# Vipermaseg/libagmv

Measured on AMD Instinct MI355X. Metric: frames/s encode+decode (AGMV hot path: quantise+classify+assemble, parse+reconstruct), synthetic, higher is better.
Workload: dtype u8; 1 GPU; c3: 1024-frame 1920x1080 agmv_synth_v1, HIGH_QUALITY palette, OPT_III (512 colours); frames_per_gpu=1024, width=1920, height=1080, palette=512 colours, reference histogram build (GPU histogram + host pick), parallelism=1024 frames per rank, 1 rank(s), no data-path collective

## Files before the change

libagmv_amd/csrc/agmv_decode_hip.hip:

```cpp
#include <hip/hip_runtime.h>

#include <stdint.h>
#include <stdlib.h>
#include <string.h>
#include <type_traits>

#include "agmv_hip_impl.h"

#ifndef DEC_T_OVERRIDE
#define DEC_T_OVERRIDE 256
#endif
constexpr int DEC_T = DEC_T_OVERRIDE;
#ifndef DEC_BPB
#define DEC_BPB 24
#endif
constexpr int DEC_STAGE = DEC_T * DEC_BPB;
constexpr int DEC_SR = DEC_STAGE / 4 / DEC_T;
constexpr int DEC_MAX_SLICES = 32;

struct dec_ws {
	uint32_t* d_dirty;
	size_t dirty_cap;
	bool dep_split;
	uint32_t* d_parse_ws;
	size_t parse_ws_cap;
	uint32_t* d_fp_ws;
	size_t fp_ws_cap;
	uint32_t* d_fp_fstate;
	uint32_t fp_frames;
	uint32_t* d_nent_own;
	size_t nent_cap;
	hipStream_t aux_stream;
	hipEvent_t ev_fork;
	hipEvent_t ev_slice[DEC_MAX_SLICES];
};

static dec_ws* dec_area(agmv_hip_ctx* c) { return (dec_ws*)c->ws[AREA_DEC]; }

static void dec_free(void* p)
{
	dec_ws* d = (dec_ws*)p;
	(void)hipFree(d->d_dirty); (void)hipFree(d->d_parse_ws); (void)hipFree(d->d_fp_ws); (void)hipFree(d->d_nent_own);
	if (d->ev_fork) (void)hipEventDestroy(d->ev_fork);
	for (int i = 0; i < DEC_MAX_SLICES; i++) if (d->ev_slice[i]) (void)hipEventDestroy(d->ev_slice[i]);
	if (d->aux_stream) (void)hipStreamDestroy(d->aux_stream);
	free(d);
}

static int need_dec_ctx(agmv_hip_ctx* c, bool palette)
{
	if (agmv_hip_enter(c, palette)) return -1;
	return palette && !agmv_hip_area(c, AREA_DEC, sizeof(dec_ws), dec_free) ? -1 : 0;
}

template <class F>
static void dec_flags(F&& f) { f(); }
template <class F, class... Rest>
static void dec_flags(F&& f, bool flag, Rest... rest) { dec_flags([&](auto... r_) { if (flag) f(std::true_type(), r_...); else f(std::false_type(), r_...); }, rest...); }
#define DEC_LAUNCH(k, grid, block, s, A, ...) do { \
	dec_flags([&](auto... b_) { hipLaunchKernelGGL((k<decltype(b_)::value...>), grid, block, 0, s, A); }, __VA_ARGS__); \
	CK(hipGetLastError()); } while (0)

__device__ __forceinline__ bool is_flag(uint32_t b) { return b == FILL_FLAG || b == NORMAL_FLAG || b == COPY_FLAG; }

struct ByteSrc {
	const uint8_t* p;
	uint32_t cap;
	__device__ __forceinline__ uint32_t operator()(uint32_t pos) const { return pos < cap ? p[pos] : 0u; }
};

struct StagedSrc {
	const __attribute__((address_space(3))) uint8_t* lds;
	uint32_t lo, len;
	const uint8_t* p;
	uint32_t cap;
	__device__ __forceinline__ uint32_t operator()(uint32_t pos) const
	{
		const uint32_t d = pos - lo;
		if (d < len) return lds[d];
		return pos < cap ? p[pos] : 0u;
	}
};

__global__ __launch_bounds__(64) void k_parse_serial(const uint8_t* __restrict__ bits, unsigned long long stride,
                                                     const uint32_t* __restrict__ bpos_a, uint32_t n_frames,
                                                     uint32_t nblk, int mode512, uint32_t* __restrict__ offsets,
                                                     uint32_t* __restrict__ nentered)
{
	uint32_t f = blockIdx.x * 64u + threadIdx.x;
	if (f >= n_frames) return;
	ByteSrc src{bits + (size_t)f * stride, (uint32_t)stride};
	const uint32_t bpos = bpos_a[f];
	uint32_t* off = offsets + (size_t)f * nblk;
	uint32_t bitpos = 0, k = 0;
	bool escape = false;
	while (k < nblk && !escape) {
		if (bitpos > bpos) break;
		off[k++] = bitpos;
		uint32_t byte = src(bitpos++);
		bool invalid = false;
		while (!is_flag(byte)) {
			byte = src(bitpos++);
			if (bitpos > bpos) { escape = true; break; }
		}
		if (!is_flag(byte)) invalid = true;
		if (byte == FILL_FLAG) {
			uint32_t idx = src(bitpos++);
			if (mode512 && (idx & 0x7fu) == 127u) bitpos++;
			if (bitpos > bpos) escape = true;
		} else if (byte == COPY_FLAG) {
		} else {
			for (int j = 0; j < 4; j++)
				for (int i = 0; i < 4; i++) {
					uint32_t idx = src(bitpos++);
					if (mode512 && (idx & 0x7fu) == 127u) bitpos++;
					if (bitpos > bpos || invalid) { escape = true; invalid = false; break; }
				}
		}
	}
	nentered[f] = k;
}

constexpr int PC = 512;
constexpr int PNSEG = PC / 64;
#ifndef PEL_OVERRIDE
#define PEL_OVERRIDE 3
#endif
constexpr int PCL = 3;
constexpr int PEL = PEL_OVERRIDE;
constexpr int PHALO = 64;
constexpr uint32_t J_EXIT = 0x8000u;
constexpr uint32_t J_END = 0xFFFFu;
constexpr uint32_t X_END = 63u;

constexpr int FC = 64;
constexpr int FH = 4;
constexpr int FOWN = 64 - FH - 1;
constexpr int FRB = FOWN * FC;

struct ParseArgs {
	const uint8_t* bits;
	unsigned long long stride;
	const uint32_t* bpos;
	uint32_t cpf;
	uint16_t* summ;
	uint32_t* centry;
	uint32_t* offsets;
	uint32_t* nentered;
	uint32_t n_frames, nblk;
	const uint32_t* fstate;
	const uint32_t* nbad;
	unsigned long long* vm;
	uint32_t maxR;
};
constexpr uint32_t FS_OK = 0, FS_TODO = 1, FS_BAD = 2;

__device__ __forceinline__ uint32_t parse_nch(const ParseArgs& A, uint32_t f, uint32_t bpos)
{
	return (!A.fstate || A.fstate[f] == FS_BAD) ? (bpos + PC) / PC : 0u;
}

__device__ __forceinline__ void wave_lds_sync()
{
	__builtin_amdgcn_fence(__ATOMIC_ACQ_REL, "wavefront");
	__builtin_amdgcn_wave_barrier();
}

template <int NLV>
struct ParseLds {
	uint8_t b[PC + PHALO];
	unsigned long long esc[PNSEG + 2];
	uint16_t jl[NLV][PC];
};

constexpr int PCD = ((PC + PHALO) / 4 + 63) / 64;

__device__ __forceinline__ void load_chunk(uint32_t (&raw)[PCD], const uint8_t* fbits, uint32_t cap, uint32_t cs, int lane)
{
#pragma unroll
	for (int q = 0; q < PCD; q++) {
		const uint32_t pos = cs + 4u * (uint32_t)(q * 64 + lane);
		raw[q] = (q * 64 + lane < (PC + PHALO) / 4 && pos < cap) ? *(const uint32_t*)(fbits + pos) : 0u;
	}
}

template <bool M512, int NLV>
__device__ __forceinline__ uint32_t parse_chunk_nodes(ParseLds<NLV>& S, uint16_t* rank_at, uint16_t* npos, uint16_t* eo, uint16_t* n0,
                                                      const uint32_t (&raw)[PCD], uint32_t bpos, uint32_t cs, int lane)
{
#pragma unroll
	for (int q = 0; q < PCD; q++) {
		const int i = q * 64 + lane;
		if (i < (PC + PHALO) / 4) ((uint32_t*)S.b)[i] = raw[q];
	}
	wave_lds_sync();
// ... 1026 lines not shown
			for (int k = 0; k < 16; k++) icol[k] = cur[k];
			istale = stale;
		}
		anystale |= stale != 0;
		if (!needfix) depstale |= stale != 0;
		if (valid) store_block(A.out + (size_t)f * npx, poff, A.w, cur);
	}
	if (valid && (anystale || needfix)) {
		if (group != 0 || needfix) {
			atomicOr(A.dirty + (blk >> 5), 1u << (blk & 31u));
			A.dirty[(A.nblk + 31) >> 5] = 1u;
		}
		if (group == 0 && depstale) A.dirty[((A.nblk + 31) >> 5) + 1] = 1u;
	}
	if (!LOOP) break;
	item += gridDim.x;
	if (item >= A.n_items) break;
	__syncthreads();
	}
}

template <bool M512, bool BM>
__global__ __launch_bounds__(64) void k_fixup(DecArgs A)
{
	__shared__ uint32_t s_pal[512];
	const int lane = threadIdx.x;
	const uint32_t npx = A.w * A.h;
	const uint32_t nwords = (A.nblk + 31) >> 5;
	if (A.dirty[nwords] == 0) return;
	const uint32_t base = blockIdx.x * 64u;
	const uint32_t w0 = A.dirty[base >> 5], w1 = (base >> 5) + 1 < nwords ? A.dirty[(base >> 5) + 1] : 0u;
	if ((w0 | w1) == 0) return;
	uint32_t blk = base + (uint32_t)lane;
	bool active = blk < A.nblk && (((lane < 32 ? w0 : w1) >> (lane & 31)) & 1u);
	const uint32_t last = A.nblk - 1;
	const bool have_last = last >= base && last < base + 64 && ((((last - base) < 32 ? w0 : w1) >> ((last - base) & 31)) & 1u);
	int nb_lane = -1;
	if (have_last && A.nblk >= 2) {
		if (last > base) { nb_lane = (int)(last - base) - 1; if (lane == nb_lane) active = true; }
		else { nb_lane = 1; if (lane == 1) { blk = last - 1; active = true; } }
	}
	for (int i = lane; i < 512; i += 64) s_pal[i] = A.pal[i];
	__syncthreads();
	if (!active) blk = 0;
	const uint32_t by = blk / A.bw, bx = blk - by * A.bw;
	const uint32_t poff = by * 4 * A.w + bx * 4;
	const bool is_last = active && blk == last;
	uint32_t cur[16], icol[16];
	if (A.prev) load_block(A.prev, poff, A.w, cur);
	else {
#pragma unroll
		for (int k = 0; k < 16; k++) cur[k] = 0;
	}
	if (A.prev_iframe) load_block(A.prev_iframe, poff, A.w, icol);
	else {
#pragma unroll
		for (int k = 0; k < 16; k++) icol[k] = 0;
	}
	uint32_t stale = 0xFFFFu, istale = 0xFFFFu;
	bool dep = false;
	for (uint32_t f = 0; f < A.n_frames; f++) {
		bool fill_written = false;
		const uint32_t own3 = cur[3], own3s = (stale >> 3) & 1u;
		if (active && blk < A.nentered[f]) {
			ByteSrc src{A.bits + (size_t)f * A.stride, (uint32_t)A.stride};
			const uint32_t o = BM ? bm_offset_of(A.vm, A.kb, A.maxR, A.bpos[f], f, blk) : A.offsets[(size_t)f * A.nblk + blk];
			decode_block<M512>(src, o, A.bpos[f], s_pal, cur, icol, istale, stale, fill_written);
		}
		const int nbl = nb_lane < 0 ? 0 : nb_lane;
		const uint32_t left = (uint32_t)__builtin_amdgcn_readlane((int)cur[7], nbl);
		const uint32_t lefts = ((uint32_t)__builtin_amdgcn_readlane((int)stale, nbl) >> 7) & 1u;
		if (is_last && fill_written) {
			const uint32_t c = A.bw == 1 ? own3 : left;
#pragma unroll
			for (int k = 0; k < 16; k++) cur[k] = c;
			stale = (A.bw == 1 ? own3s : lefts) ? 0xFFFFu : 0u;
		}
		if (((A.first_fc + f) & 3u) == 0) {
#pragma unroll
			for (int k = 0; k < 16; k++) icol[k] = cur[k];
			istale = stale;
		}
		if (active) store_block(A.out + (size_t)f * npx, poff, A.w, cur);
		if (active && stale) dep = true;
	}
	if (dep) A.dirty[nwords + 1] = 1u;
}

static int check_slab(const uint8_t* d_bits, size_t stride)
{
	if ((stride & 3u) || stride < 4 || ((uintptr_t)d_bits & 3u)) return agmv_hip_err("agmv_hip: bitstream slab and stride must be 4-byte aligned");
	return 0;
}

struct DecRows {
	const uint8_t* bits;
	size_t stride;
	const uint32_t* bpos;
	uint32_t *offsets, *nentered;
	uint32_t n_frames, nblk;
};
static DecRows rows_range(DecRows r, uint32_t f0, uint32_t f1)
{
	r.bits += (size_t)f0 * r.stride; r.bpos += f0; r.nentered += f0; r.n_frames = f1 - f0;
	if (r.offsets) r.offsets += (size_t)f0 * r.nblk;
	return r;
}
struct DecPix {
	uint32_t w, h, first_fc;
	uint32_t* out;
	const uint32_t *prev, *prev_iframe;
};

static uint32_t dirty_words(uint32_t nblk) { return (nblk + 31) / 32 + 2; }

enum ParseMode { PARSE_FAST, PARSE_ROBUST, PARSE_SERIAL };
static ParseMode parse_mode()
{
	const char* m = getenv("AGMV_HIP_PARSE");
	return !m ? PARSE_FAST : strcmp(m, "robust") == 0 ? PARSE_ROBUST : strcmp(m, "serial") == 0 ? PARSE_SERIAL : PARSE_FAST;
}

static uint32_t parse_grid_x(agmv_hip_ctx* c, uint32_t n_frames, size_t cap)
{
	uint32_t gx = (uint32_t)(((size_t)c->n_cu * 512 + n_frames - 1) / n_frames);
	if (gx < 32) gx = 32;
	if (gx > 256) gx = 256;
	if (gx > cap) gx = (uint32_t)cap;
	return gx < 1 ? 1 : gx;
}

static int parse_launch_robust(agmv_hip_ctx* c, const DecRows& r, size_t ws_frames, hipStream_t s,
                               const uint32_t* fstate, const uint32_t* nbad, unsigned long long* vm, uint32_t maxR)
{
	const size_t cpf = (r.stride + PC) / PC, maxchunks = cpf * ws_frames;
	if (maxchunks >> 32) return agmv_hip_err("agmv_hip: parser batch too large (%zu chunk rows)", maxchunks);
	dec_ws* d = dec_area(c);
	CK(agmv_hip_dev_grow(&d->d_parse_ws, &d->parse_ws_cap, (maxchunks + (maxchunks * 33 + 1) / 2 + 16) * 4, 1));
	ParseArgs A;
	memset(&A, 0, sizeof(A));
	A.bits = r.bits; A.stride = r.stride; A.bpos = r.bpos; A.offsets = r.offsets; A.nentered = r.nentered;
	A.cpf = (uint32_t)cpf; A.centry = d->d_parse_ws; A.summ = (uint16_t*)(A.centry + maxchunks);
	A.n_frames = r.n_frames; A.nblk = r.nblk; A.fstate = fstate; A.vm = vm; A.maxR = maxR; A.nbad = nbad;
	const uint32_t n = r.n_frames;
	const dim3 grid(parse_grid_x(c, n, fstate && cpf > 32 ? 32 : cpf), fstate ? (n < 64u ? n : 64u) : (n < 65535u ? n : 65535u));
	const int m512 = c->mode512;
	DEC_LAUNCH(k_parse_chunks, grid, dim3(64), s, A, m512);
	hipLaunchKernelGGL(k_parse_stitch, dim3(fstate ? (n < 1024u ? n : 1024u) : n), dim3(64), 0, s, A);
	CK(hipGetLastError());
	DEC_LAUNCH(k_parse_emit, grid, dim3(64), s, A, m512);
	return 0;
}

static int parse_launch(agmv_hip_ctx* c, const DecRows& r, size_t ws_frames, hipStream_t s, DecArgs* bm)
{
	const bool robust_only = parse_mode() == PARSE_ROBUST;
	const uint32_t n_frames = r.n_frames;
	dec_ws* d = dec_area(c);
	d->d_fp_fstate = nullptr; d->fp_frames = 0;
	if (!bm && (n_frames > 65535u || robust_only)) return parse_launch_robust(c, r, ws_frames, s, nullptr, nullptr, nullptr, 0);
	if (n_frames > 65535u) return agmv_hip_err("agmv_hip: more than 65535 frames in one parser launch");
	const size_t maxR = (r.stride + FRB - 1) / FRB + 1, nreg = maxR * ws_frames;
	const uint32_t tpfd = (r.nblk + DEC_T - 1) / DEC_T;
	const size_t b_rec = nreg * sizeof(uint4), b_vm = nreg * FOWN * 8, b_kb = nreg * 4, b_fs = ((ws_frames * 4 + 15) & ~(size_t)15);
	const size_t b_tx = bm ? (((size_t)ws_frames * (tpfd + 1) * 4 + 15) & ~(size_t)15) : 0;
	CK(agmv_hip_dev_grow(&d->d_fp_ws, &d->fp_ws_cap, b_rec + b_vm + b_kb + b_fs + b_tx + 16, 1));
	FpArgs A;
	memset(&A, 0, sizeof(A));
	A.bits = r.bits; A.stride = r.stride; A.bpos = r.bpos; A.offsets = r.offsets; A.nentered = r.nentered;
	uint8_t* w = (uint8_t*)d->d_fp_ws;
	A.rec = (uint4*)w; A.vm = (unsigned long long*)(w + b_rec); A.kb = (uint32_t*)(w + b_rec + b_vm); A.fstate = (uint32_t*)(w + b_rec + b_vm + b_kb);
	A.tidx = bm ? (uint32_t*)(w + b_rec + b_vm + b_kb + b_fs) : nullptr; A.tpfd = tpfd;
	A.nbad = (uint32_t*)(w + b_rec + b_vm + b_kb + b_fs + b_tx);
	A.n_frames = n_frames; A.nblk = r.nblk; A.maxR = (uint32_t)maxR;
	if (bm) { A.dirty = bm->dirty; A.ndirty = dirty_words(r.nblk); }
	uint32_t gx = parse_grid_x(c, n_frames, maxR);
	uint32_t gy = n_frames;
	if ((size_t)gx * gy > 131072u) {
		const uint32_t want = (uint32_t)(((size_t)r.stride / 8 + FRB - 1) / FRB) + 1;
		if (gx > want) gx = want;
		if ((size_t)gx * gy > 131072u) gy = 131072u / gx;
	}
	const dim3 grid(gx, gy);
	if (robust_only) {
		CK(hipMemsetAsync(A.tidx, 0xFF, (size_t)n_frames * (tpfd + 1) * 4, s));
		CK(hipMemsetAsync(A.vm, 0, (size_t)n_frames * maxR * FOWN * 8, s));
		CK(hipMemsetD32Async((hipDeviceptr_t)A.fstate, (int)FS_BAD, n_frames, s));
		CK(hipMemsetD32Async((hipDeviceptr_t)A.nbad, (int)n_frames, 1, s));
	} else {
		DEC_LAUNCH(k_fp_walk, grid, dim3(64), s, A, c->mode512);
		DEC_LAUNCH(k_fp_finish, dim3(n_frames), dim3(64), s, A, c->mode512);
	}
	d->d_fp_fstate = A.fstate; d->fp_frames = n_frames;
	if (!bm) {
		hipLaunchKernelGGL(k_fp_expand, dim3(gx, n_frames), dim3(64), 0, s, A);
		CK(hipGetLastError());
		return parse_launch_robust(c, r, ws_frames, s, A.fstate, A.nbad, nullptr, 0);
	}
	bm->vm = A.vm; bm->kb = A.kb; bm->tidx = A.tidx; bm->maxR = A.maxR;
	if (parse_launch_robust(c, r, ws_frames, s, A.fstate, A.nbad, A.vm, A.maxR)) return -1;
	hipLaunchKernelGGL(k_fp_tiles, dim3(gx / 2 ? gx / 2 : 1, gy), dim3(64), 0, s, A);
	CK(hipGetLastError());
	return 0;
}

extern "C" int agmv_hip_parse_frames_dev(agmv_hip_ctx* c, const uint8_t* d_bits, size_t stride, const uint32_t* d_bpos,
                                         uint32_t n_frames, uint32_t w, uint32_t h, uint32_t* d_offsets, uint32_t* d_nentered,
                                         void* stream)
{
	if (need_dec_ctx(c, true)) return -1;
	if (agmv_hip_check_geometry(w, h)) return -1;
	if (n_frames == 0) return 0;
	const DecRows r = {d_bits, stride, d_bpos, d_offsets, d_nentered, n_frames, (w / 4) * (h / 4)};
	hipStream_t s = (hipStream_t)stream;
	if (parse_mode() == PARSE_SERIAL) {
		hipLaunchKernelGGL(k_parse_serial, dim3((n_frames + 63) / 64), dim3(64), 0, s, d_bits,
		                   (unsigned long long)stride, d_bpos, n_frames, r.nblk, c->mode512, d_offsets, d_nentered);
		CK(hipGetLastError());
		return 0;
	}
	if (check_slab(d_bits, stride)) return -1;
	agmv_hip_ev_mark(c, 2, s);
	if (parse_launch(c, r, n_frames, s, nullptr)) return -1;
	agmv_hip_ev_mark(c, 3, s);
	return 0;
}

extern "C" int agmv_hip_parse_fallback_frames(agmv_hip_ctx* c, void* stream)
{
	if (need_dec_ctx(c, false)) return -1;
	const dec_ws* d = dec_area(c);
	if (!d || !d->d_fp_fstate || d->fp_frames == 0) return 0;
	CK(hipStreamSynchronize((hipStream_t)stream));
	uint32_t* h = (uint32_t*)malloc((size_t)d->fp_frames * 4);
	if (!h) return agmv_hip_err("agmv_hip: out of host memory");
	if (hipMemcpy(h, d->d_fp_fstate, (size_t)d->fp_frames * 4, hipMemcpyDeviceToHost) != hipSuccess) { free(h); agmv_hip_err("agmv_hip: D2H failed"); return -1; }
	int n = 0;
	for (uint32_t i = 0; i < d->fp_frames; i++) n += h[i] != FS_OK;
	free(h);
	return n;
}

static int decode_prepare(agmv_hip_ctx* c, DecArgs& A, const DecRows& r, const DecPix& px, hipStream_t s, bool clear)
{
	if (((uintptr_t)px.out & 15u) || ((uintptr_t)px.prev & 15u) || ((uintptr_t)px.prev_iframe & 15u)) return agmv_hip_err("agmv_hip: pixel buffers must be 16-byte aligned");
	if (check_slab(r.bits, r.stride)) return -1;
	memset(&A, 0, sizeof(A));
	A.bits = r.bits; A.stride = r.stride; A.bpos = r.bpos; A.offsets = r.offsets; A.nentered = r.nentered;
	A.out = px.out; A.pal = c->d_pal; A.prev = px.prev; A.prev_iframe = px.prev_iframe;
	A.n_frames = r.n_frames; A.w = px.w; A.h = px.h; A.bw = px.w / 4; A.nblk = r.nblk;
	A.tpf = (A.nblk + DEC_T - 1) / DEC_T;
	A.first_fc = px.first_fc; A.phase = px.first_fc & 3u; A.n_groups = (r.n_frames + A.phase + 3) / 4;
	const size_t nwords = dirty_words(A.nblk);
	dec_ws* d = dec_area(c);
	CK(agmv_hip_dev_grow(&d->d_dirty, &d->dirty_cap, (nwords + 1) * 4, 1));
	A.dirty = d->d_dirty; d->dep_split = false;
	if (clear) CK(hipMemsetAsync(d->d_dirty, 0, nwords * 4, s));
	return 0;
}

static int decode_launch(agmv_hip_ctx* c, DecArgs A, uint32_t g0, uint32_t g1, hipStream_t s)
{
	A.grp0 = g0; A.n_items = (g1 - g0) * A.tpf;
	uint32_t nwg = A.n_items;
	if (const char* e = getenv("AGMV_DEC_GRID")) {
		const long n = atol(e);
		if (n > 0 && (unsigned long)n < nwg) nwg = (uint32_t)n;
	}
	DEC_LAUNCH(k_decode, dim3(nwg), dim3(DEC_T), s, A, c->mode512, A.vm != nullptr, nwg < A.n_items);
	return 0;
}

static int fixup_launch(agmv_hip_ctx* c, const DecArgs& A, hipStream_t s)
{
	DEC_LAUNCH(k_fixup, dim3((A.nblk + 63) / 64), dim3(64), s, A, c->mode512, A.vm != nullptr);
	return 0;
}

extern "C" int agmv_hip_decode_frames_dev(agmv_hip_ctx* c, const uint8_t* d_bits, size_t stride, const uint32_t* d_bpos,
                                          const uint32_t* d_offsets, const uint32_t* d_nentered, uint32_t n_frames,
                                          uint32_t w, uint32_t h, uint32_t first_fc, uint32_t* d_out,
                                          const uint32_t* d_prev, const uint32_t* d_prev_iframe, void* stream)
{
	if (need_dec_ctx(c, true)) return -1;
	if (agmv_hip_check_geometry(w, h)) return -1;
	if (n_frames == 0) return 0;
	hipStream_t s = (hipStream_t)stream;
	const DecRows r = {d_bits, stride, d_bpos, const_cast<uint32_t*>(d_offsets), const_cast<uint32_t*>(d_nentered), n_frames, (w / 4) * (h / 4)};
	const DecPix px = {w, h, first_fc, d_out, d_prev, d_prev_iframe};
	DecArgs A;
	if (decode_prepare(c, A, r, px, s, true)) return -1;
	agmv_hip_ev_mark(c, 4, s);
	if (decode_launch(c, A, 0, A.n_groups, s)) return -1;
	if (fixup_launch(c, A, s)) return -1;
	agmv_hip_ev_mark(c, 5, s);
	return 0;
}

extern "C" int agmv_hip_parse_decode_frames_dev(agmv_hip_ctx* c, const uint8_t* d_bits, size_t stride, const uint32_t* d_bpos,
                                                uint32_t n_frames, uint32_t w, uint32_t h, uint32_t first_fc,
                                                uint32_t* d_offsets, uint32_t* d_nentered, uint32_t* d_out,
                                                const uint32_t* d_prev, const uint32_t* d_prev_iframe, void* stream)
{
	if (need_dec_ctx(c, true)) return -1;
	if (agmv_hip_check_geometry(w, h)) return -1;
	if (n_frames == 0) return 0;
	hipStream_t s = (hipStream_t)stream;
	const DecRows r = {d_bits, stride, d_bpos, d_offsets, d_nentered, n_frames, (w / 4) * (h / 4)};
	const DecPix px = {w, h, first_fc, d_out, d_prev, d_prev_iframe};
	DecArgs A;
	if (decode_prepare(c, A, r, px, s, true)) return -1;
	uint32_t nsl = 1;
	if (getenv("AGMV_DEC_SLICES")) nsl = (uint32_t)atoi(getenv("AGMV_DEC_SLICES"));
	if (nsl > A.n_groups) nsl = A.n_groups;
	if (nsl > (uint32_t)DEC_MAX_SLICES) nsl = DEC_MAX_SLICES;
	if (nsl < 1) nsl = 1;
	const uint32_t gps = (A.n_groups + nsl - 1) / nsl;
	auto first_frame = [&](uint32_t g) -> uint32_t { const long f = (long)g * 4 - (long)A.phase; return f < 0 ? 0u : ((uint32_t)f > n_frames ? n_frames : (uint32_t)f); };
	const size_t ws_frames = (size_t)gps * 4;
	agmv_hip_ev_mark(c, 6, s);
	if (nsl == 1) {
		if (parse_launch(c, r, n_frames, s, nullptr)) return -1;
		if (decode_launch(c, A, 0, A.n_groups, s)) return -1;
	} else {
		dec_ws* d = dec_area(c);
		if (!d->aux_stream) {
			CK(hipStreamCreateWithFlags(&d->aux_stream, hipStreamNonBlocking));
			CK(hipEventCreateWithFlags(&d->ev_fork, hipEventDisableTiming));
			for (int i = 0; i < DEC_MAX_SLICES; i++) CK(hipEventCreateWithFlags(&d->ev_slice[i], hipEventDisableTiming));
		}
		CK(hipEventRecord(d->ev_fork, s));
		CK(hipStreamWaitEvent(d->aux_stream, d->ev_fork, 0));
		uint32_t k = 0;
		for (uint32_t g0 = 0; g0 < A.n_groups; g0 += gps, k++) {
			const uint32_t g1 = g0 + gps < A.n_groups ? g0 + gps : A.n_groups;
			if (parse_launch(c, rows_range(r, first_frame(g0), first_frame(g1)), ws_frames, d->aux_stream, nullptr)) return -1;
			CK(hipEventRecord(d->ev_slice[k], d->aux_stream));
			CK(hipStreamWaitEvent(s, d->ev_slice[k], 0));
			if (decode_launch(c, A, g0, g1, s)) return -1;
		}
	}
	if (fixup_launch(c, A, s)) return -1;
	agmv_hip_ev_mark(c, 7, s);
	return 0;
}

extern "C" int agmv_hip_decode_bitstreams_dev(agmv_hip_ctx* c, const uint8_t* d_bits, size_t stride, const uint32_t* d_bpos,
                                              uint32_t n_frames, uint32_t w, uint32_t h, uint32_t first_fc,
                                              uint32_t* d_nentered, uint32_t* d_out,
                                              const uint32_t* d_prev, const uint32_t* d_prev_iframe, void* stream)
{
	if (need_dec_ctx(c, true)) return -1;
	if (agmv_hip_check_geometry(w, h)) return -1;
	if (n_frames == 0) return 0;
	hipStream_t s = (hipStream_t)stream;
	dec_ws* d = dec_area(c);
	if (!d_nentered) {
		CK(agmv_hip_dev_grow(&d->d_nent_own, &d->nent_cap, (size_t)n_frames * 4, 1));
		d_nentered = d->d_nent_own;
	}
	const DecRows all = {d_bits, stride, d_bpos, nullptr, d_nentered, n_frames, (w / 4) * (h / 4)};
	const size_t npx = (size_t)w * h;
	constexpr uint32_t PART = 65532u;
	agmv_hip_ev_mark(c, 6, s);
	for (uint32_t f0 = 0; f0 < n_frames;) {
		uint32_t f1 = n_frames;
		if (f1 - f0 > PART) { f1 = f0 + PART; f1 -= (first_fc + f1) & 3u; }
		const DecRows r = rows_range(all, f0, f1);
		const DecPix px = {w, h, first_fc + f0, d_out + (size_t)f0 * npx, f0 == 0 ? d_prev : d_out + (size_t)(f0 - 1) * npx,
		                   f0 == 0 ? d_prev_iframe : d_out + (size_t)(f0 - 4) * npx};
		DecArgs A;
		if (decode_prepare(c, A, r, px, s, false)) return -1;
		agmv_hip_ev_mark(c, 2, s);
		if (parse_launch(c, r, r.n_frames, s, &A)) return -1;
		agmv_hip_ev_mark(c, 3, s);
		agmv_hip_ev_mark(c, 4, s);
		if (decode_launch(c, A, 0, A.n_groups, s)) return -1;
		if (fixup_launch(c, A, s)) return -1;
		agmv_hip_ev_mark(c, 5, s);
		if (f0 == 0 && f1 < n_frames) {
			const size_t dw = (A.nblk + 31) / 32 + 1;
			CK(hipMemcpyAsync(d->d_dirty + dw + 1, d->d_dirty + dw, 4, hipMemcpyDeviceToDevice, s));
		}
		f0 = f1;
	}
	d->dep_split = n_frames > PART;
	agmv_hip_ev_mark(c, 7, s);
	return 0;
}

extern "C" int agmv_hip_decode_prior_dependent(agmv_hip_ctx* c, uint32_t w, uint32_t h, void* stream)
{
	if (need_dec_ctx(c, false)) return -1;
	const dec_ws* d = dec_area(c);
	if (!d || !d->d_dirty) return agmv_hip_err("agmv_hip: no decode has run on this context");
	const size_t nblk = (size_t)(w / 4) * (h / 4);
	uint32_t v = 0;
	CK(hipStreamSynchronize((hipStream_t)stream));
	CK(hipMemcpy(&v, d->d_dirty + (nblk + 31) / 32 + (d->dep_split ? 2 : 1), 4, hipMemcpyDeviceToHost));
	return v ? 1 : 0;
}

extern "C" int agmv_hip_decode_frames(agmv_hip_ctx* c, const uint8_t* h_bits, size_t stride, const uint32_t* h_bpos,
                                      uint32_t n_frames, uint32_t w, uint32_t h, uint32_t first_fc, uint32_t* h_out,
                                      const uint32_t* h_prev, const uint32_t* h_prev_iframe)
{
	if (need_dec_ctx(c, true)) return -1;
	if (agmv_hip_check_geometry(w, h)) return -1;
	if (n_frames == 0) return 0;
	const size_t npx = (size_t)w * h, nblk = npx / 16;
	uint8_t* d_bits = nullptr;
	uint32_t *d_bpos = nullptr, *d_off = nullptr, *d_ne = nullptr, *d_out = nullptr, *d_prev = nullptr, *d_pi = nullptr;
	int rc = -1;
	do {
		if (hipMalloc(&d_bits, stride * n_frames) != hipSuccess || hipMalloc(&d_bpos, 4 * (size_t)n_frames) != hipSuccess ||
		    hipMalloc(&d_off, 4 * nblk * n_frames) != hipSuccess || hipMalloc(&d_ne, 4 * (size_t)n_frames) != hipSuccess ||
		    hipMalloc(&d_out, 4 * npx * n_frames) != hipSuccess || (h_prev && hipMalloc(&d_prev, 4 * npx) != hipSuccess) ||
		    (h_prev_iframe && hipMalloc(&d_pi, 4 * npx) != hipSuccess)) {
			agmv_hip_err("agmv_hip: device allocation failed"); break;
		}
		if (hipMemcpy(d_bits, h_bits, stride * n_frames, hipMemcpyHostToDevice) != hipSuccess ||
		    hipMemcpy(d_bpos, h_bpos, 4 * (size_t)n_frames, hipMemcpyHostToDevice) != hipSuccess ||
		    (h_prev && hipMemcpy(d_prev, h_prev, 4 * npx, hipMemcpyHostToDevice) != hipSuccess) ||
		    (h_prev_iframe && hipMemcpy(d_pi, h_prev_iframe, 4 * npx, hipMemcpyHostToDevice) != hipSuccess)) {
			agmv_hip_err("agmv_hip: H2D failed"); break;
		}
		if (agmv_hip_parse_frames_dev(c, d_bits, stride, d_bpos, n_frames, w, h, d_off, d_ne, nullptr)) break;
		if (agmv_hip_decode_frames_dev(c, d_bits, stride, d_bpos, d_off, d_ne, n_frames, w, h, first_fc, d_out, d_prev, d_pi, nullptr)) break;
		if (hipMemcpy(h_out, d_out, 4 * npx * n_frames, hipMemcpyDeviceToHost) != hipSuccess) { agmv_hip_err("agmv_hip: D2H failed"); break; }
		rc = 0;
	} while (0);
	(void)hipFree(d_bits); (void)hipFree(d_bpos); (void)hipFree(d_off); (void)hipFree(d_ne); (void)hipFree(d_out); (void)hipFree(d_prev); (void)hipFree(d_pi);
	return rc;
}
```

libagmv_amd/csrc/agmv_hip.hip:

```cpp
#include <hip/hip_runtime.h>

#include <stdarg.h>
#include <stdint.h>
#include <stdio.h>
#include <stdlib.h>
#include <string.h>
#include <pthread.h>

#include "agmv_hip_impl.h"

static thread_local char g_err[512] = "";

int agmv_hip_err(const char* fmt, ...)
{
	va_list ap;
	va_start(ap, fmt);
	vsnprintf(g_err, sizeof(g_err), fmt, ap);
	va_end(ap);
	return -1;
}

int agmv_hip_hip_failed(const char* what, hipError_t e, const char* file, int line)
{
	return agmv_hip_err("agmv_hip: %s failed: %s (%s:%d)", what, hipGetErrorString(e), file, line);
// ... 610 lines not shown
						n += (e2 >> 8) & 1u;
						*(u16u*)(sp + n + (2 + 2 * m)) = (uint16_t)(w >> 16);
						n += e2 >> 24;
					}
				} else {
#pragma unroll
					for (int m = 0; m < 4; m++)
						*(u32u*)(sp + 1 + 4 * m) = __builtin_amdgcn_perm(ep[2 * m + 1], ep[2 * m], 0x06040200u);
				}
			} else if (fill) {
				if (M512) {
					const uint32_t idx = e0 & 0xffu, p7 = (e0 >> 1) & 0x80u;
					*(u16u*)(sp + 1) = (uint16_t)(p7 | (idx < 127u ? idx : 127u) | (idx << 8));
				} else {
					sp[1] = (uint8_t)e0;
				}
			}
			asm volatile("" ::: "memory");
			sp[0] = copy ? COPY_FLAG : (fill ? FILL_FLAG : NORMAL_FLAG);
		}
		if (have_prev) copy_out_prev();
		prefetch_next();

		have_prev = true; p_tile = g.tile; p_f = f; p_len = wtot;
		it++;
		pre_next = ST_PREFIX;
		if (wave == (int)(it % ENC_WAVES) && p_tile != 0) pre_next = st_load(A.status + (size_t)p_f * A.tpf, (int)p_tile - 1 - lane);
		new_tile = advance(cur, false);
		return true;
	};
	for (;;) {
#pragma unroll
		for (int d = 0; d < ENC_PFDEPTH; d++)
			if (!body(pxs[d])) goto done;
	}
done:;
}

__global__ __launch_bounds__(64) void k_encode_verdict(const uint32_t* __restrict__ ctrl, uint32_t* __restrict__ sizes, uint32_t n_frames)
{
	if (ctrl[1] == 0) return;
	for (uint32_t f = threadIdx.x; f < n_frames; f += 64) sizes[f] = 0xFFFFFFFFu;
}

__global__ __launch_bounds__(64) void k_nearest_direct(const uint32_t* __restrict__ pal, int mode512, const uint32_t* __restrict__ pix,
                                                       size_t n, uint16_t* __restrict__ out)
{
	const size_t i = (size_t)blockIdx.x * 64 + threadIdx.x;
	if (i >= n) return;
	const uint32_t c = pix[i];
	const int r = (int)((c >> 16) & 0xff), g = (int)((c >> 8) & 0xff), b = (int)(c & 0xff);
	uint32_t d0, i0;
	nearest_in(pal, r, g, b, d0, i0);
	uint32_t e = i0;
	if (mode512) {
		uint32_t d1, i1;
		nearest_in(pal + 256, r, g, b, d1, i1);
		if (!(d0 <= d1)) e = 0x100u | i1;
	}
	out[i] = (uint16_t)e;
}

__global__ __launch_bounds__(64) void k_within2_count(const uint32_t* __restrict__ ab, uint32_t* __restrict__ out)
{
	const int lane = threadIdx.x;
	const bool in = lane < 16 && within2(ab[lane], ab[16 + lane]);
	const unsigned long long m = __ballot(in);
	if (lane == 0) out[0] = (uint32_t)__popcll(m);
}

struct lut_share {
	int device, mode512, refs;
	uint32_t pal[512];
	uint16_t* d_lut;
	uint32_t* d_mtx;
	uint32_t* d_pal;
	hipEvent_t built;
	lut_share* next;
};
static pthread_mutex_t g_lut_mu = PTHREAD_MUTEX_INITIALIZER;
static lut_share* g_luts = nullptr;

static void lut_release(lut_share* sh)
{
	if (!sh) return;
	pthread_mutex_lock(&g_lut_mu);
	if (--sh->refs == 0) {
		for (lut_share** pp = &g_luts; *pp; pp = &(*pp)->next)
			if (*pp == sh) { *pp = sh->next; break; }
		(void)hipFree(sh->d_lut); (void)hipFree(sh->d_mtx); (void)hipFree(sh->d_pal);
		if (sh->built) (void)hipEventDestroy(sh->built);
		free(sh);
	}
	pthread_mutex_unlock(&g_lut_mu);
}

extern "C" int agmv_hip_device_count(void)
{
	int n = 0;
	if (hipGetDeviceCount(&n) != hipSuccess) return 0;
	return n;
}

extern "C" void agmv_hip_destroy(agmv_hip_ctx* c);
extern "C" agmv_hip_ctx* agmv_hip_create(int device)
{
	int n = 0;
	hipError_t e = hipGetDeviceCount(&n);
	if (e != hipSuccess || n <= 0) {
		agmv_hip_err("agmv_hip: no HIP device available (%s); the AGMV hot path has no CPU fallback",
		             e == hipSuccess ? "device count 0" : hipGetErrorString(e));
		return nullptr;
	}
	if (device < 0 || device >= n) {
		agmv_hip_err("agmv_hip: device %d out of range (0..%d)", device, n - 1);
		return nullptr;
	}
	CKP(hipSetDevice(device));
	agmv_hip_ctx* c = (agmv_hip_ctx*)calloc(1, sizeof(*c));
	if (!c) { agmv_hip_err("agmv_hip: out of host memory"); return nullptr; }
	c->device = device;
	hipDeviceProp_t prop;
	hipError_t e2 = hipMalloc(&c->d_ctrl, CTRL_BYTES);
	if (e2 == hipSuccess) e2 = hipMemset(c->d_ctrl, 0, CTRL_BYTES);
	if (e2 == hipSuccess) e2 = hipStreamSynchronize(nullptr);
	if (e2 == hipSuccess) e2 = hipGetDeviceProperties(&prop, device);
	if (e2 != hipSuccess) {
		agmv_hip_hip_failed("agmv_hip_create", e2, __FILE_NAME__, __LINE__);
		agmv_hip_destroy(c);
		return nullptr;
	}
	c->n_cu = prop.multiProcessorCount;
	{
		int per_cu = 0;
		const size_t lds = (size_t)512 * MROW * 4 + ENC_LDS_EXTRA;
		(void)hipFuncSetAttribute((const void*)k_encode<true, false>, hipFuncAttributeMaxDynamicSharedMemorySize, (int)lds);
		if (hipOccupancyMaxActiveBlocksPerMultiprocessor(&per_cu, (const void*)k_encode<true, false>, ENC_T, lds) != hipSuccess || per_cu < 1) per_cu = 2;
		if (getenv("AGMV_HIP_DEBUG")) fprintf(stderr, "agmv_hip: k_encode: %d workgroup(s) of %d lanes resident per CU (%zu B of LDS each), %d CUs\n", per_cu, ENC_T, lds, c->n_cu);
		c->enc_grid = prop.multiProcessorCount * per_cu;
	}
	return c;
}

extern "C" void agmv_hip_destroy(agmv_hip_ctx* c)
{
	if (!c) return;
	(void)hipSetDevice(c->device);
	lut_release(c->share);
	(void)hipFree(c->d_ctrl);
	(void)hipFree(c->d_status); (void)hipFree(c->d_ient_tmp);
	(void)hipFree(c->d_nn_pal); (void)hipFree(c->d_nn_pix); (void)hipFree(c->d_nn_ent);
	if (c->ev_enc) (void)hipEventDestroy(c->ev_enc);
	for (int i = 0; i < 8; i++) if (c->ev[i]) (void)hipEventDestroy(c->ev[i]);
	for (int k = 0; k < AREA_KINDS; k++) if (c->ws[k]) c->ws_free[k](c->ws[k]);
	free(c);
}

void* agmv_hip_area(agmv_hip_ctx* c, agmv_hip_area_kind kind, size_t bytes, void (*destroy)(void*))
{
	if (!c->ws[kind]) {
		if (!(c->ws[kind] = calloc(1, bytes))) { agmv_hip_err("agmv_hip: out of host memory"); return nullptr; }
		c->ws_free[kind] = destroy;
	}
	return c->ws[kind];
}

void agmv_hip_ev_mark(agmv_hip_ctx* c, int which, hipStream_t s)
{
	if (c->timing) (void)hipEventRecord(c->ev[which], s);
}

extern "C" int agmv_hip_enable_timing(agmv_hip_ctx* c, int on)
{
	if (!c) return -1;
	CK(hipSetDevice(c->device));
	if (on && !c->ev[0]) for (int i = 0; i < 8; i++) CK(hipEventCreate(&c->ev[i]));
	c->timing = on ? 1 : 0;
	return 0;
}

extern "C" float agmv_hip_last_kernel_ms(agmv_hip_ctx* c, int which)
{
	float ms = -1.0f;
	if (!c || !c->timing || which < 0 || which > 3) return -1.0f;
	if (hipEventSynchronize(c->ev[2 * which + 1]) != hipSuccess) return -1.0f;
	if (hipEventElapsedTime(&ms, c->ev[2 * which], c->ev[2 * which + 1]) != hipSuccess) return -1.0f;
	return ms;
}

int agmv_hip_enter(agmv_hip_ctx* c, bool palette)
{
	if (!c) return agmv_hip_err("agmv_hip: NULL context");
	if (palette && !c->have_palette) return agmv_hip_err("agmv_hip: agmv_hip_set_palette was not called");
	CK(hipSetDevice(c->device));
	return 0;
}

extern "C" int agmv_hip_set_palette(agmv_hip_ctx* c, const uint32_t p0[256], const uint32_t p1[256], int mode512, void* stream)
{
	if (agmv_hip_enter(c)) return -1;
	hipStream_t s = (hipStream_t)stream;
	uint32_t pal[512];
	memcpy(pal, p0, 1024);
	if (p1) memcpy(pal + 256, p1, 1024); else memset(pal + 256, 0, 1024);
	mode512 = mode512 ? 1 : 0;
	pthread_mutex_lock(&g_lut_mu);
	lut_share* sh = nullptr;
	for (lut_share* q = g_luts; q; q = q->next)
		if (q->device == c->device && q->mode512 == mode512 && memcmp(q->pal, pal, sizeof(pal)) == 0) { sh = q; break; }
	int rc = 0;
	if (sh) sh->refs++;
	else {
		sh = (lut_share*)calloc(1, sizeof(*sh));
		hipError_t e = sh ? hipSuccess : hipErrorOutOfMemory;
		if (e == hipSuccess) e = hipMalloc(&sh->d_lut, (size_t)LUT_ENTRIES * sizeof(uint16_t));
		if (e == hipSuccess) e = hipMalloc(&sh->d_mtx, 512 * MROW * sizeof(uint32_t));
		if (e == hipSuccess) e = hipMalloc(&sh->d_pal, 512 * sizeof(uint32_t));
		if (e == hipSuccess) e = hipEventCreateWithFlags(&sh->built, hipEventDisableTiming);
		if (e == hipSuccess) e = hipMemcpyAsync(sh->d_pal, pal, sizeof(pal), hipMemcpyHostToDevice, s);
		if (e == hipSuccess) e = hipStreamSynchronize(s);
		if (e == hipSuccess) {
			hipLaunchKernelGGL(k_lut_build, dim3(LUT_COLOURS / 256), dim3(256), 0, s, sh->d_pal, mode512, sh->d_lut);
			e = hipGetLastError();
		}
		if (e == hipSuccess) {
			hipLaunchKernelGGL(k_mtx_build, dim3((512 * MROW + 255) / 256), dim3(256), 0, s, sh->d_pal, sh->d_mtx);
			e = hipGetLastError();
		}
		if (e == hipSuccess) e = hipEventRecord(sh->built, s);
		if (e != hipSuccess) {
			rc = agmv_hip_hip_failed("agmv_hip_set_palette", e, __FILE_NAME__, __LINE__);
			if (sh) { (void)hipFree(sh->d_lut); (void)hipFree(sh->d_mtx); (void)hipFree(sh->d_pal); if (sh->built) (void)hipEventDestroy(sh->built); free(sh); }
			sh = nullptr;
		} else {
			sh->device = c->device; sh->mode512 = mode512; sh->refs = 1;
			memcpy(sh->pal, pal, sizeof(pal));
			sh->next = g_luts; g_luts = sh;
		}
	}
	pthread_mutex_unlock(&g_lut_mu);
	if (rc) return rc;
	if (hipStreamWaitEvent(s, sh->built, 0) != hipSuccess) { lut_release(sh); return agmv_hip_hip_failed("hipStreamWaitEvent", hipErrorUnknown, __FILE_NAME__, __LINE__); }
	lut_share* old_sh = c->share;
	c->share = sh; c->d_lut = sh->d_lut; c->d_mtx = sh->d_mtx; c->d_pal = sh->d_pal;
	c->mode512 = mode512;
	c->have_palette = 1;
	if (old_sh) {
		CK(hipDeviceSynchronize());
		lut_release(old_sh);
	}
	return 0;
}

extern "C" int agmv_hip_quantise_dev(agmv_hip_ctx* c, const uint32_t* d_pix, size_t n, uint16_t* d_entries, void* stream)
{
	if (agmv_hip_enter(c, true)) return -1;
	if (n == 0) return 0;
	size_t blocks = (n + 255) / 256;
	if (blocks > 8192) blocks = 8192;
	hipLaunchKernelGGL(k_quantise, dim3((unsigned)blocks), dim3(256), 0, (hipStream_t)stream, d_pix, n, c->d_lut, d_entries);
	CK(hipGetLastError());
	return 0;
}

extern "C" int agmv_hip_dither_frames_async(agmv_hip_ctx* c, uint32_t strength, uint32_t* d_pix, uint32_t w, uint32_t h, uint32_t n_frames,
                                            void* stream)
{
	if (agmv_hip_enter(c, true)) return -1;
	if (!d_pix || ((uintptr_t)d_pix & 3u)) return agmv_hip_err("agmv_hip: dither: d_pix must be a 4-byte aligned device pointer");
	if (strength < 1 || strength > 64) return agmv_hip_err("agmv_hip: dither: strength must be 1 .. 64 (got %u)", strength);
	if (w == 0 || h == 0) return agmv_hip_err("agmv_hip: dither: width/height must be non-zero (got %ux%u)", w, h);
	if ((uint64_t)w * h >= (1ull << 31)) return agmv_hip_err("agmv_hip: dither: a frame must have fewer than 2^31 pixels (got %ux%u)", w, h);
	if (n_frames == 0) return 0;
	const uint32_t npx = w * h, cap = (uint32_t)(c->n_cu * DITHER_WG_PER_CU);
	uint32_t gx = (npx + DITHER_T - 1) / DITHER_T, gy = 1;
	if (gx > cap) gx = cap;
	else { gy = cap / gx; if (gy > n_frames) gy = n_frames; if (gy > 65535u) gy = 65535u; }
	hipLaunchKernelGGL(k_dither, dim3(gx, gy), dim3(DITHER_T), 0, (hipStream_t)stream, d_pix, w, npx, n_frames, (int)strength, c->d_lut, c->d_pal);
	CK(hipGetLastError());
	return 0;
}

int agmv_hip_check_geometry(uint32_t w, uint32_t h)
{
	if (w == 0 || h == 0 || (w & 3u) || (h & 3u))
		return agmv_hip_err("agmv_hip: width/height must be non-zero multiples of 4 (got %ux%u); "
		                    "the reference's block loops have no edge handling (src/agmv_encode.c:365-366)", w, h);
	if ((uint64_t)w * h >= (1ull << 31)) return agmv_hip_err("agmv_hip: frame too large");
	return 0;
}

static int encode_dev(agmv_hip_ctx* c, const uint32_t* d_pix, uint32_t n_frames, uint32_t w, uint32_t h,
                      uint32_t first_fc, uint8_t* d_out, size_t out_stride, uint32_t* d_sizes,
                      uint16_t* d_ientries, void* stream, bool entries)
{
	if (agmv_hip_enter(c, true)) return -1;
	if (agmv_hip_check_geometry(w, h)) return -1;
	if (n_frames == 0) return 0;
	if (out_stride < agmv_hip_max_usize(w, h, c->mode512))
		return agmv_hip_err("agmv_hip: out_stride %zu < agmv_hip_max_usize %zu", out_stride, agmv_hip_max_usize(w, h, c->mode512));
	if (((uintptr_t)d_pix & 15u) || ((uintptr_t)d_out & 3u)) return agmv_hip_err("agmv_hip: d_pix must be 16-byte and d_out 4-byte aligned");
	hipStream_t s = (hipStream_t)stream;
	EncArgs A;
	memset(&A, 0, sizeof(A));
	A.pix = d_pix; A.out = d_out; A.sizes = d_sizes; A.lut = c->d_lut; A.mtx = c->d_mtx; A.ientries_in = d_ientries; A.ientries_out = d_ientries;
	A.out_stride = out_stride;
	A.n_frames = n_frames; A.w = w; A.h = h; A.bw = w / 4; A.nblk = (w / 4) * (h / 4);
	A.tpf = (A.nblk + ENC_T - 1) / ENC_T;
	A.first_fc = first_fc; A.phase = first_fc & 3u;
	A.n_groups = (n_frames + A.phase + 3) / 4;
	A.total_tiles = A.n_groups * A.tpf;
	if (A.phase != 0 && !d_ientries)
		return agmv_hip_err("agmv_hip: batch starts inside a GOP (frame_count %u) but no I-frame entries were supplied", first_fc);
	A.last_iframe = 0xffffffffu;
	for (int64_t f = (int64_t)n_frames - 1; f >= 0; f--)
		if (((first_fc + (uint32_t)f) & 3u) == 0) { A.last_iframe = (uint32_t)f; break; }
	size_t need = (size_t)n_frames * A.tpf;
	CK(agmv_hip_dev_grow(&c->d_status, &c->status_cap, need));
	A.status = c->d_status; A.ctrl = c->d_ctrl;
	const bool ient_both = d_ientries && A.phase != 0 && A.last_iframe != 0xffffffffu;
	const size_t npx_e = (size_t)w * h;
	if (ient_both) {
		CK(agmv_hip_dev_grow(&c->d_ient_tmp, &c->ient_cap, npx_e));
		A.ientries_out = c->d_ient_tmp;
	}
	if (!c->ev_enc) CK(hipEventCreateWithFlags(&c->ev_enc, hipEventDisableTiming));
	if (c->have_enc && c->enc_stream != s) CK(hipStreamWaitEvent(s, c->ev_enc, 0));
	CK(hipMemsetAsync(c->d_status, 0, need * sizeof(unsigned long long), s));
	CK(hipMemsetAsync(c->d_ctrl, 0, CTRL_BYTES, s));
	uint32_t grid = (uint32_t)c->enc_grid;
	if (grid > A.total_tiles) grid = A.total_tiles;
	const size_t lds = (size_t)(c->mode512 ? 512 : 256) * MROW * 4 + ENC_LDS_EXTRA;
	void (*kern)(EncArgs) = c->mode512 ? (entries ? k_encode<true, true> : k_encode<true, false>)
	                                   : (entries ? k_encode<false, true> : k_encode<false, false>);
	CK(hipFuncSetAttribute((const void*)kern, hipFuncAttributeMaxDynamicSharedMemorySize, (int)lds));
	agmv_hip_ev_mark(c, 0, s);
	hipLaunchKernelGGL(kern, dim3(grid), dim3(ENC_T), lds, s, A);
	agmv_hip_ev_mark(c, 1, s);
	CK(hipGetLastError());
// ... 276 lines not shown
```

libagmv_amd/csrc/agmv_hip_impl.h:

```cpp
#pragma once
#include <hip/hip_runtime.h>

#include <stddef.h>
#include <stdint.h>

#include "../../include/agmv_hip.h"

enum agmv_hip_area_kind { AREA_DEC, AREA_LZSS, AREA_LZ77, AREA_LZ_DECODE, AREA_PALETTE, AREA_KINDS };

struct agmv_hip_ctx {
	int device;
	int mode512;
	int have_palette;
	uint16_t* d_lut;
	uint32_t* d_mtx;
	uint32_t* d_pal;
	struct lut_share* share;
	unsigned long long* d_status;
	size_t status_cap;
	uint32_t* d_ctrl;
	uint16_t* d_ient_tmp;
	size_t ient_cap;
	int enc_grid;
	int n_cu;
	int timing;
	hipEvent_t ev[8];
	hipEvent_t ev_enc;
	hipStream_t enc_stream;
	int have_enc;
	uint32_t* d_nn_pal;
	uint32_t* d_nn_pix;
	uint16_t* d_nn_ent;
	size_t nn_cap;
	void* ws[AREA_KINDS];
	void (*ws_free[AREA_KINDS])(void*);
};

int agmv_hip_err(const char* fmt, ...) __attribute__((format(printf, 1, 2)));
int agmv_hip_hip_failed(const char* what, hipError_t e, const char* file, int line);
#define CK(x) do { hipError_t e_ = (x); if (e_ != hipSuccess) return agmv_hip_hip_failed(#x, e_, __FILE_NAME__, __LINE__); } while (0)
#define CKP(x) do { hipError_t e_ = (x); if (e_ != hipSuccess) { agmv_hip_hip_failed(#x, e_, __FILE_NAME__, __LINE__); return nullptr; } } while (0)

int agmv_hip_enter(agmv_hip_ctx* c, bool palette = false);

void* agmv_hip_area(agmv_hip_ctx* c, agmv_hip_area_kind kind, size_t bytes, void (*destroy)(void*));

void agmv_hip_ev_mark(agmv_hip_ctx* c, int which, hipStream_t s);
int agmv_hip_check_geometry(uint32_t w, uint32_t h);

template <class T>
static inline hipError_t agmv_hip_dev_grow(T** p, size_t* cap, size_t need, size_t unit = sizeof(T))
{
	if (cap && need <= *cap) return hipSuccess;
	if (cap) *cap = 0;
	hipError_t e = hipFree(*p);
	*p = nullptr;
	if (e == hipSuccess) e = hipMalloc((void**)p, need * unit);
	if (e == hipSuccess && cap) *cap = need;
	return e;
}

#define FILL_FLAG   0x4Eu
#define NORMAL_FLAG 0x2Fu
#define COPY_FLAG   0x5Eu
#define FILL_COUNT  14u
#define COPY_COUNT  13u

__device__ __forceinline__ void lds_barrier()
{
	asm volatile("s_waitcnt lgkmcnt(0)\n\ts_barrier" ::: "memory");
}

template <int CTRL, int ROW_MASK>
__device__ __forceinline__ uint32_t dpp_or0(uint32_t x)
{
	return (uint32_t)__builtin_amdgcn_update_dpp(0, (int)x, CTRL, ROW_MASK, 0xF, false);
}

__device__ __forceinline__ uint32_t wave_incl_scan(uint32_t x, int)
{
	x += dpp_or0<0x111, 0xF>(x);
	x += dpp_or0<0x112, 0xF>(x);
	x += dpp_or0<0x114, 0xF>(x);
	x += dpp_or0<0x118, 0xF>(x);
	x += dpp_or0<0x142, 0xA>(x);
	x += dpp_or0<0x143, 0xC>(x);
	return x;
}

__device__ __forceinline__ uint32_t wave_sum(uint32_t x)
{
	return (uint32_t)__builtin_amdgcn_readlane((int)wave_incl_scan(x, 0), 63);
}
```

Baseline: 214,800 frames/s.

## Split bitstream decode into bounded frame ranges sized by pixel footprint

Decode now processes frames in ranges whose size is derived from a fixed pixel-byte budget (or an env override) instead of the near-65535 partition limit. Frame state is kept in one per-call buffer so the ranges chain correctly, and per-range timing events are added. The aim is to bound the parser and decode workspace and keep the working set smaller. The cost is more kernel launches and serialisation across ranges.

```diff
diff --git a/libagmv_amd/csrc/agmv_decode_hip.hip b/libagmv_amd/csrc/agmv_decode_hip.hip
--- a/libagmv_amd/csrc/agmv_decode_hip.hip
+++ b/libagmv_amd/csrc/agmv_decode_hip.hip
@@ -28,6 +28,8 @@
 	size_t fp_ws_cap;
 	uint32_t* d_fp_fstate;
 	uint32_t fp_frames;
+	uint32_t* d_fstate_call;
+	size_t fstate_call_cap;
 	uint32_t* d_nent_own;
 	size_t nent_cap;
 	hipStream_t aux_stream;
@@ -41,6 +43,7 @@
 {
 	dec_ws* d = (dec_ws*)p;
 	(void)hipFree(d->d_dirty); (void)hipFree(d->d_parse_ws); (void)hipFree(d->d_fp_ws); (void)hipFree(d->d_nent_own);
+	(void)hipFree(d->d_fstate_call);
 	if (d->ev_fork) (void)hipEventDestroy(d->ev_fork);
 	for (int i = 0; i < DEC_MAX_SLICES; i++) if (d->ev_slice[i]) (void)hipEventDestroy(d->ev_slice[i]);
 	if (d->aux_stream) (void)hipStreamDestroy(d->aux_stream);
@@ -1373,7 +1376,7 @@
 	return 0;
 }
 
-static int parse_launch(agmv_hip_ctx* c, const DecRows& r, size_t ws_frames, hipStream_t s, DecArgs* bm)
+static int parse_launch(agmv_hip_ctx* c, const DecRows& r, size_t ws_frames, hipStream_t s, DecArgs* bm, uint32_t* fstate = nullptr)
 {
 	const bool robust_only = parse_mode() == PARSE_ROBUST;
 	const uint32_t n_frames = r.n_frames;
@@ -1391,6 +1394,7 @@
 	A.bits = r.bits; A.stride = r.stride; A.bpos = r.bpos; A.offsets = r.offsets; A.nentered = r.nentered;
 	uint8_t* w = (uint8_t*)d->d_fp_ws;
 	A.rec = (uint4*)w; A.vm = (unsigned long long*)(w + b_rec); A.kb = (uint32_t*)(w + b_rec + b_vm); A.fstate = (uint32_t*)(w + b_rec + b_vm + b_kb);
+	if (fstate) A.fstate = fstate;
 	A.tidx = bm ? (uint32_t*)(w + b_rec + b_vm + b_kb + b_fs) : nullptr; A.tpfd = tpfd;
 	A.nbad = (uint32_t*)(w + b_rec + b_vm + b_kb + b_fs + b_tx);
 	A.n_frames = n_frames; A.nblk = r.nblk; A.maxR = (uint32_t)maxR;
@@ -1566,6 +1570,21 @@
 	return 0;
 }
 
+constexpr uint32_t DEC_PART_MAX = 65532u;
+constexpr size_t DEC_RANGE_PIXEL_BYTES = (size_t)512 * 1920 * 1080 * 4;
+static uint32_t dec_range_frames(uint32_t w, uint32_t h)
+{
+	size_t n = DEC_PART_MAX;
+	if (const char* e = getenv("AGMV_DEC_RANGE_FRAMES")) {
+		const long v = atol(e);
+		if (v > 0) n = ((size_t)v + 3) & ~(size_t)3;
+	} else if (DEC_RANGE_PIXEL_BYTES) {
+		const size_t gops = DEC_RANGE_PIXEL_BYTES / ((size_t)w * h * 16);
+		n = (gops ? gops : 1) * 4;
+	}
+	return n < DEC_PART_MAX ? (uint32_t)n : DEC_PART_MAX;
+}
+
 extern "C" int agmv_hip_decode_bitstreams_dev(agmv_hip_ctx* c, const uint8_t* d_bits, size_t stride, const uint32_t* d_bpos,
                                               uint32_t n_frames, uint32_t w, uint32_t h, uint32_t first_fc,
                                               uint32_t* d_nentered, uint32_t* d_out,
@@ -1582,30 +1601,42 @@
 	}
 	const DecRows all = {d_bits, stride, d_bpos, nullptr, d_nentered, n_frames, (w / 4) * (h / 4)};
 	const size_t npx = (size_t)w * h;
-	constexpr uint32_t PART = 65532u;
+	const uint32_t range = dec_range_frames(w, h);
+	const bool cut = n_frames > range;
+	const size_t ws_frames = (size_t)range + 3;
+	uint32_t* fstate = nullptr;
+	if (cut) {
+		CK(agmv_hip_dev_grow(&d->d_fstate_call, &d->fstate_call_cap, (size_t)n_frames * 4, 1));
+		fstate = d->d_fstate_call;
+	}
 	agmv_hip_ev_mark(c, 6, s);
-	for (uint32_t f0 = 0; f0 < n_frames;) {
+	int k = 0;
+	for (uint32_t f0 = 0; f0 < n_frames; k++) {
 		uint32_t f1 = n_frames;
-		if (f1 - f0 > PART) { f1 = f0 + PART; f1 -= (first_fc + f1) & 3u; }
+		if (f1 - f0 > range) {
+			f1 = f0 + range; f1 -= (first_fc + f1) & 3u;
+			if (f1 < 4) f1 = f1 + 4 < n_frames ? f1 + 4 : n_frames;
+		}
 		const DecRows r = rows_range(all, f0, f1);
 		const DecPix px = {w, h, first_fc + f0, d_out + (size_t)f0 * npx, f0 == 0 ? d_prev : d_out + (size_t)(f0 - 1) * npx,
 		                   f0 == 0 ? d_prev_iframe : d_out + (size_t)(f0 - 4) * npx};
 		DecArgs A;
 		if (decode_prepare(c, A, r, px, s, false)) return -1;
-		agmv_hip_ev_mark(c, 2, s);
-		if (parse_launch(c, r, r.n_frames, s, &A)) return -1;
-		agmv_hip_ev_mark(c, 3, s);
-		agmv_hip_ev_mark(c, 4, s);
+		if (agmv_hip_ev_mark_range(c, 2, k, s)) return -1;
+		if (parse_launch(c, r, cut ? ws_frames : r.n_frames, s, &A, fstate ? fstate + f0 : nullptr)) return -1;
+		if (agmv_hip_ev_mark_range(c, 3, k, s)) return -1;
+		if (agmv_hip_ev_mark_range(c, 4, k, s)) return -1;
 		if (decode_launch(c, A, 0, A.n_groups, s)) return -1;
 		if (fixup_launch(c, A, s)) return -1;
-		agmv_hip_ev_mark(c, 5, s);
-		if (f0 == 0 && f1 < n_frames) {
+		if (agmv_hip_ev_mark_range(c, 5, k, s)) return -1;
+		if (f0 == 0 && cut) {
 			const size_t dw = (A.nblk + 31) / 32 + 1;
 			CK(hipMemcpyAsync(d->d_dirty + dw + 1, d->d_dirty + dw, 4, hipMemcpyDeviceToDevice, s));
 		}
 		f0 = f1;
 	}
-	d->dep_split = n_frames > PART;
+	d->dep_split = cut;
+	if (cut) { d->d_fp_fstate = fstate; d->fp_frames = n_frames; }
 	agmv_hip_ev_mark(c, 7, s);
 	return 0;
 }
diff --git a/libagmv_amd/csrc/agmv_hip.hip b/libagmv_amd/csrc/agmv_hip.hip
--- a/libagmv_amd/csrc/agmv_hip.hip
+++ b/libagmv_amd/csrc/agmv_hip.hip
@@ -786,6 +786,8 @@
 	(void)hipFree(c->d_nn_pal); (void)hipFree(c->d_nn_pix); (void)hipFree(c->d_nn_ent);
 	if (c->ev_enc) (void)hipEventDestroy(c->ev_enc);
 	for (int i = 0; i < 8; i++) if (c->ev[i]) (void)hipEventDestroy(c->ev[i]);
+	for (int i = 0; i < 4 * c->ev_rng_cap; i++) (void)hipEventDestroy(c->ev_rng[i]);
+	free(c->ev_rng);
 	for (int k = 0; k < AREA_KINDS; k++) if (c->ws[k]) c->ws_free[k](c->ws[k]);
 	free(c);
 }
@@ -801,7 +803,26 @@
 
 void agmv_hip_ev_mark(agmv_hip_ctx* c, int which, hipStream_t s)
 {
-	if (c->timing) (void)hipEventRecord(c->ev[which], s);
+	if (!c->timing) return;
+	if (which == 2 || which == 4) c->ev_rng_n[which / 2 - 1] = 0;
+	(void)hipEventRecord(c->ev[which], s);
+}
+
+int agmv_hip_ev_mark_range(agmv_hip_ctx* c, int which, int range, hipStream_t s)
+{
+	if (!c->timing) return 0;
+	if (range == 0) { agmv_hip_ev_mark(c, which, s); return 0; }
+	if (range > c->ev_rng_cap) {
+		const int cap = range > 2 * c->ev_rng_cap ? range : 2 * c->ev_rng_cap;
+		hipEvent_t* p = (hipEvent_t*)realloc(c->ev_rng, (size_t)cap * 4 * sizeof(hipEvent_t));
+		if (!p) return agmv_hip_err("agmv_hip: out of host memory");
+		c->ev_rng = p;
+		for (; c->ev_rng_cap < cap; c->ev_rng_cap++)
+			for (int i = 0; i < 4; i++) CK(hipEventCreate(&p[4 * c->ev_rng_cap + i]));
+	}
+	CK(hipEventRecord(c->ev_rng[4 * (range - 1) + which - 2], s));
+	if (which == 2 || which == 4) c->ev_rng_n[which / 2 - 1] = range;
+	return 0;
 }
 
 extern "C" int agmv_hip_enable_timing(agmv_hip_ctx* c, int on)
@@ -819,6 +840,13 @@
 	if (!c || !c->timing || which < 0 || which > 3) return -1.0f;
 	if (hipEventSynchronize(c->ev[2 * which + 1]) != hipSuccess) return -1.0f;
 	if (hipEventElapsedTime(&ms, c->ev[2 * which], c->ev[2 * which + 1]) != hipSuccess) return -1.0f;
+	if (which == 1 || which == 2)
+		for (int k = 0; k < c->ev_rng_n[which - 1]; k++) {
+			hipEvent_t* e = c->ev_rng + 4 * k + 2 * (which - 1);
+			float part = 0.0f;
+			if (hipEventSynchronize(e[1]) != hipSuccess || hipEventElapsedTime(&part, e[0], e[1]) != hipSuccess) return -1.0f;
+			ms += part;
+		}
 	return ms;
 }
 
diff --git a/libagmv_amd/csrc/agmv_hip_impl.h b/libagmv_amd/csrc/agmv_hip_impl.h
--- a/libagmv_amd/csrc/agmv_hip_impl.h
+++ b/libagmv_amd/csrc/agmv_hip_impl.h
@@ -25,6 +25,9 @@
 	int n_cu;
 	int timing;
 	hipEvent_t ev[8];
+	hipEvent_t* ev_rng;
+	int ev_rng_cap;
+	int ev_rng_n[2];
 	hipEvent_t ev_enc;
 	hipStream_t enc_stream;
 	int have_enc;
@@ -46,6 +49,7 @@
 void* agmv_hip_area(agmv_hip_ctx* c, agmv_hip_area_kind kind, size_t bytes, void (*destroy)(void*));
 
 void agmv_hip_ev_mark(agmv_hip_ctx* c, int which, hipStream_t s);
+int agmv_hip_ev_mark_range(agmv_hip_ctx* c, int which, int range, hipStream_t s);
 int agmv_hip_check_geometry(uint32_t w, uint32_t h);
 
 template <class T>
```

Measured after the change: 219,700 frames/s, median of 6. 2.3% higher.
